# josebeo2016/SCL-Deepfake-audio-detection

Hardware: AMD Instinct MI355X
Metric: train-step utterances/sec (64000-sample clips) (higher is better)
Workload: dtype bf16

## Files before the change

### include/scl_hip.h

```cpp
#ifndef SCL_HIP_H
#define SCL_HIP_H
#include <stdint.h>
#include <stddef.h>

#ifdef __cplusplus
extern "C" {
#endif

#define SCL_OK            0
#define SCL_EINVAL       -1
#define SCL_ELAUNCH      -2
#define SCL_EUNSUPPORTED -3

int         scl_version(void);
const char* scl_last_error(void);

int scl_stream_wait_stream(void* waiter, void* signaler);

#define SCL_KID_GEMM 0
#define SCL_KID_GEMM_F32 2
#define SCL_KID_AUG  1
#define SCL_KID_MAX  8
int scl_build_flags(void);
int scl_prof_enable(int kid, int on);
// ... 45 lines not shown
    const float* bias;
    int64_t c_bs1, c_bs2;
    int64_t c_rbstride;
    int64_t c_split_stride;
    int64_t bias_bs2;
    int32_t c_rpb, ldc;
    int32_t M, N, K;
    int32_t nb1, nb2, splitk;
    int32_t flags;
    float    alpha;
    float    drop_p;
    uint32_t drop_seed;
    int32_t  _pad;
    float*   colsum_part;
} SclGemmDesc;

int scl_gemm_bf16(const SclGemmDesc* desc, void* stream);
int scl_gemm_bf16_group_ok(const SclGemmDesc* descs, int n);
int scl_gemm_bf16_group(const SclGemmDesc* descs, int n, void* stream);
int scl_gemm_bf16_group_tiles(const SclGemmDesc* desc);
int scl_gemm_bf16_group_part(const SclGemmDesc* descs, const int32_t* tile0, const int32_t* ntile, int n, void* stream);

int scl_gemm_uses_wide_tiles(const SclGemmDesc* desc);
int scl_gemm_colsum_rows(const SclGemmDesc* desc);

int scl_posconv_supported(int T, int K, int G, int Cg);
int scl_posconv_wgrad_supported(int T, int K, int G, int Cg);
int scl_posconv_wgrad(const void* dypad, int dy_row0, const void* xpad, float* dw, int B, int T, int K, int G, int Cg, void* stream);
int scl_posconv_mfma(const void* xpad, const void* w, float* C, const float* bias, void* c2, const float* R, int B, int T, int K, int G,
                     int Cg, int fwd, void* stream);

int scl_debug_gemm_stamps(unsigned long long* out, int nblocks);
long long scl_debug_gemm_persistent_launches(void);

int scl_gemm_splitk_finish(const SclGemmDesc* desc, const float* slabs, int nslabs, int64_t stride, void* stream);

int scl_reduce_slabs_f32(const float* slabs, float* out, int64_t n, int nslabs, int64_t stride, void* stream);
#define SCL_SLAB_MAX_JOBS 8
typedef struct SclSlabJob {
    const float* slabs;
    float*       out;
    int64_t      n, stride;
    int32_t      nslabs, _pad;
} SclSlabJob;
int scl_reduce_slabs_multi(const SclSlabJob* jobs, int njobs, void* stream);

int scl_bn_nslabs(int N);
int scl_bn_fwd(const float* x, int N, int C, const float* gamma, const float* beta, float* running_mean, float* running_var,
               long long* num_batches_tracked, int training, float momentum, float eps, int act, float* part, float* mean,
               float* rstd, float* y, void* y2, int y2_bf16, int m_W, int m_HW, int64_t m_bs, int64_t m_rs, int64_t m_cs,
               int64_t m_base, void* stream);
int scl_bn_bwd(const float* dy, const float* y, const float* x, const float* mean, const float* rstd, const float* gamma, int N, int C,
               int act, int training, float* part, float* sums, float* dgamma, float* dbeta, float* dx, int accumulate, void* stream);
int scl_bn_eval_masked(const float* x, int B, int H, int W, int C, const float* gamma, const float* beta, const float* running_mean,
                       const float* running_var, float eps, int act, const int32_t* valid, float* mean, float* rstd, float* y, void* stream);
int scl_bn_eval_cols(const float* x, int B, int H, int W, int C, const float* gamma, const float* beta, const float* running_mean,
                     const float* running_var, float eps, int act, const int32_t* widths, float* mean, float* rstd, float* y, void* stream);
int scl_zero_cols(float* x, int B, int H, int W, int C, const int32_t* widths, void* stream);
int scl_bn_masked_nslabs(int B, int H, int W);
int scl_bn_fwd_masked(const float* x, int B, int H, int W, int C, const float* gamma, const float* beta, float* running_mean,
                      float* running_var, long long* num_batches_tracked, float momentum, float eps, int act, const int32_t* valid,
                      const int32_t* valid_host, float* part, float* mean, float* rstd, float* y, void* stream);
int scl_bn_bwd_masked(const float* dy, const float* y, const float* x, const float* mean, const float* rstd, const float* gamma, int B,
                      int H, int W, int C, int act, const int32_t* valid, const int32_t* valid_host, float* part, float* sums,
                      float* dgamma, float* dbeta, float* dx, int accumulate, void* stream);
int scl_bn_fwd_cols(const float* x, int B, int H, int W, int C, const float* gamma, const float* beta, float* running_mean,
// ... 323 lines not shown
```

### scl-deepfake-audio-detection_amd/csrc/gemm.hip

```cpp
#include "gemm_common.h"

using namespace sclg;

namespace {

constexpr int BM = 128, BN = 128;

struct StageK {
    __amdgpu_buffer_rsrc_t rsrc;
    unsigned rowoff[4];
    unsigned lds_off[4];
    int kcur, kend;

    __device__ __forceinline__ void init(const OpK& o, const char* base, int row0, int rowlimit, int kbegin, int kend_, int tid) {
        rsrc = make_rsrc(base);
        const int c = tid & 7;
#pragma unroll
        for (int i = 0; i < 4; ++i) {
            const int row = (tid >> 3) + 32 * i;
            const int r = row0 + row;
            rowoff[i] = r < rowlimit ? row_off(o, (unsigned)r) : OOB;
            lds_off[i] = (unsigned)(row * 128 + ((c ^ ((row >> 1) & 7)) << 4));
        }
        kcur = kbegin + 8 * c; kend = kend_;
// ... 906 lines not shown
            else SCL_LAUNCH((scl_gemm_big_kernel<true, true>), bgrid, bblock, BIG_LDS, s, k);
#endif
#ifdef SCL_EXPERIMENTS
        } else if (deep) {
            static bool deep_attr_set = false;
            if (!deep_attr_set) {
                hipFuncSetAttribute((const void*)scl_gemm_deep_kernel<false, false, DEEP_S>, hipFuncAttributeMaxDynamicSharedMemorySize, DEEP_LDS);
                hipFuncSetAttribute((const void*)scl_gemm_deep_kernel<false, true, DEEP_S>, hipFuncAttributeMaxDynamicSharedMemorySize, DEEP_LDS);
                hipFuncSetAttribute((const void*)scl_gemm_deep_kernel<true, false, DEEP_S>, hipFuncAttributeMaxDynamicSharedMemorySize, DEEP_LDS);
                hipFuncSetAttribute((const void*)scl_gemm_deep_kernel<true, true, DEEP_S>, hipFuncAttributeMaxDynamicSharedMemorySize, DEEP_LDS);
                deep_attr_set = true;
            }
            if (!at && !bt) SCL_LAUNCH((scl_gemm_deep_kernel<false, false, DEEP_S>), grid, block, DEEP_LDS, s, k);
            else if (!at && bt) SCL_LAUNCH((scl_gemm_deep_kernel<false, true, DEEP_S>), grid, block, DEEP_LDS, s, k);
            else if (at && !bt) SCL_LAUNCH((scl_gemm_deep_kernel<true, false, DEEP_S>), grid, block, DEEP_LDS, s, k);
            else SCL_LAUNCH((scl_gemm_deep_kernel<true, true, DEEP_S>), grid, block, DEEP_LDS, s, k);
#endif
        } else if (dma) {
            if (!at && !bt) SCL_LAUNCH((scl_gemm_dma_kernel<false, false>), grid, block, lds, s, k);
            else if (!at && bt) SCL_LAUNCH((scl_gemm_dma_kernel<false, true>), grid, block, lds, s, k);
            else if (at && !bt) SCL_LAUNCH((scl_gemm_dma_kernel<true, false>), grid, block, lds, s, k);
            else SCL_LAUNCH((scl_gemm_dma_kernel<true, true>), grid, block, lds, s, k);
        } else {
            if (!at && !bt) SCL_LAUNCH((scl_gemm_kernel<false, false>), grid, block, lds, s, k);
            else if (!at && bt) SCL_LAUNCH((scl_gemm_kernel<false, true>), grid, block, lds, s, k);
            else if (at && !bt) SCL_LAUNCH((scl_gemm_kernel<true, false>), grid, block, lds, s, k);
            else SCL_LAUNCH((scl_gemm_kernel<true, true>), grid, block, lds, s, k);
        }
    }
    return scl_check_launch("scl_gemm_bf16");
}

extern "C" long long scl_debug_gemm_persistent_launches(void) { return scl_gemm_w8p_launches(); }
extern "C" int scl_build_flags(void) {
#ifdef SCL_EXPERIMENTS
    return 1;
#else
    return 0;
#endif
}

extern "C" int scl_debug_gemm_stamps(unsigned long long* out, int nblocks) {
    SCL_REQUIRE(out && nblocks > 0 && nblocks <= 4096, "gemm stamps: bad args");
    return scl_gemm_read_stamps(out, nblocks);
}

__global__ __launch_bounds__(256) void scl_gemm_finish_kernel(const GemmK d, const float* __restrict__ slabs, int nslabs, long long stride) {
    const int ncg = (d.N + 3) >> 2;
    const long long idx = (long long)blockIdx.x * 256 + threadIdx.x;
    if (idx >= (long long)d.M * ncg) return;
    const int row = (int)(idx / ncg), col = (int)(idx - (long long)row * ncg) * 4;
    const int flags = d.flags;
    const float* p = slabs + (long long)row * d.N + col;
    float v[4] = {0.f, 0.f, 0.f, 0.f};
    const bool full = col + 4 <= d.N && !(d.N & 3) && !(stride & 3);
    for (int s = 0; s < nslabs; ++s, p += stride) {
        if (full) {
            const float4 t = *reinterpret_cast<const float4*>(p);
            v[0] += t.x; v[1] += t.y; v[2] += t.z; v[3] += t.w;
        } else {
            for (int i = 0; i < 4; ++i) if (col + i < d.N) v[i] += p[i];
        }
    }
    const unsigned q = udiv_magic((unsigned)row, d.c_magic, d.c_shift);
    const long long off = (long long)q * d.c_rbstride + (long long)((unsigned)row - q * d.c_rpb) * d.ldc + col;
    const float* bias = (flags & SCL_GEMM_HAS_BIAS) ? d.bias : nullptr;
// ... 71 lines not shown
```

### scl-deepfake-audio-detection_amd/csrc/gemm_common.h

```cpp
#pragma once
#include "common.h"

namespace sclg {

constexpr int BK = 64;
constexpr int TILE_BYTES = 128 * 64 * 2;
constexpr unsigned OOB = 0xFFFFFFFFu;

struct OpK {
    const void* ptr;
    long long bs1, bs2;
    unsigned rb_bytes, ld_bytes, cout_bytes;
    unsigned rpb, rpb_magic, rpb_shift;
    unsigned cin, cin_magic, cin_mshift, esz_shift;
};
struct GemmK {
    OpK A, B;
    void* C; void* C2; const void* R; const float* bias; float* colsum;
    long long c_bs1, c_bs2, c_rbstride, c_split_stride, bias_bs2;
    unsigned c_rpb, c_magic, c_shift;
    int ldc, M, N, K, nb2, splitk, flags, vec_ok, group_m, tile_m, debug;
    float alpha, drop_p;
    unsigned drop_seed;
};
// ... 226 lines not shown
template <int NMT>
__device__ __forceinline__ void gemm_epilogue_blk(const GemmK& d, f32x4 (&acc)[NMT][4], int mbase, int nbase, int mlimit, int nmt,
                                                  int z1, int z2, int ksplit, int lane) {
    constexpr int KEY = SCL_GEMM_C_F32 | SCL_GEMM_C2_F32 | SCL_GEMM_R_F32 | SCL_GEMM_HAS_BIAS | SCL_GEMM_HAS_C2 | SCL_GEMM_DROPOUT |
                        (0xF << SCL_GEMM_ACT_SHIFT) | (0xF << SCL_GEMM_RMODE_SHIFT) | (0xF << SCL_GEMM_RACT_SHIFT);
    const int f = d.flags & KEY, fb = f & ~SCL_GEMM_HAS_BIAS;
    if (!(d.debug & 16)) {
        if (fb == 0) return gemm_epilogue_blk_k<NMT, 1>(d, acc, mbase, nbase, mlimit, nmt, z1, z2, ksplit, lane);
        if (f == (SCL_GEMM_HAS_BIAS | SCL_GEMM_HAS_C2 | (5 << SCL_GEMM_ACT_SHIFT))) return gemm_epilogue_blk_k<NMT, 2>(d, acc, mbase, nbase, mlimit, nmt, z1, z2, ksplit, lane);
        if (f == ((2 << SCL_GEMM_RMODE_SHIFT) | (4 << SCL_GEMM_RACT_SHIFT))) return gemm_epilogue_blk_k<NMT, 3>(d, acc, mbase, nbase, mlimit, nmt, z1, z2, ksplit, lane);
        if (fb == (SCL_GEMM_C_F32 | SCL_GEMM_R_F32 | (1 << SCL_GEMM_RMODE_SHIFT))) return gemm_epilogue_blk_k<NMT, 4>(d, acc, mbase, nbase, mlimit, nmt, z1, z2, ksplit, lane);
        if (fb == SCL_GEMM_C_F32) return gemm_epilogue_blk_k<NMT, 5>(d, acc, mbase, nbase, mlimit, nmt, z1, z2, ksplit, lane);
    }
    gemm_epilogue_blk_k<NMT, 0>(d, acc, mbase, nbase, mlimit, nmt, z1, z2, ksplit, lane);
}

__device__ __forceinline__ void gemm_epilogue(const GemmK& d, f32x4 (&acc)[4][4], int m0, int n0, int z1, int z2, int ksplit,
                                              int lane, int wr, int wc) {
    gemm_epilogue_blk<4>(d, acc, m0 + wr * 64, n0 + wc * 64, d.M, 4, z1, z2, ksplit, lane);
}





void make_magic(unsigned dv, unsigned* magic, unsigned* shift);
bool fill_operand(const SclOperand& o, const char* name, long long rows, long long contig, OpK* k, int esz);
int scl_gemm_f32_launch(const SclGemmDesc& d, GemmK& k, hipStream_t s);

struct W8Plan { int variant, tiles_m, tile_m; long long tiles, cost; int ncu = 0; };
bool scl_gemm_w8_plan(const GemmK& k, bool at, bool bt, const SclGemmDesc& d, long long zdim, int ncu, W8Plan* plan);
int scl_gemm_read_stamps(unsigned long long* out, int nblocks);
long long scl_gemm_w8p_launches();
int scl_gemm_w8_persist_blocks(const GemmK& k, bool at, bool bt, const W8Plan& plan, long long zdim);
int scl_gemm_w8_launch(GemmK& k, bool at, bool bt, const W8Plan& plan, long long zdim, hipStream_t s);
constexpr int W8_GROUP_MAX = 8;
bool scl_gemm_w8_group_member_ok(const GemmK& k, bool at, bool bt, const SclGemmDesc& d);
int scl_gemm_w8_group_tiles(const GemmK& k);
int scl_gemm_w8_group_launch(GemmK* ks, int n, const int* tile0, const int* ntile, hipStream_t s);

bool scl_gemm_x2_plan(const GemmK& k, bool at, bool bt, const SclGemmDesc& d, long long zdim, int ncu, W8Plan* plan);
int scl_gemm_x2_launch(GemmK& k, bool at, bool bt, const W8Plan& plan, long long zdim, hipStream_t s);

}
```

### scl-deepfake-audio-detection_amd/csrc/gemm_w8.hip

```cpp
#include "gemm_common.h"
#include "gemm_w8_epi.h"

using namespace sclg;

__device__ unsigned long long scl_gemm_stamps[4096 * 8];

namespace {

__device__ __forceinline__ void w8_stamp(const GemmK& d, int slot, int lane, int wave) {
    if ((d.flags & SCL_GEMM_STAMPS) && wave == 0 && lane == 0 && blockIdx.x < 4096 && blockIdx.z == 0) {
        scl_gemm_stamps[blockIdx.x * 8 + 2 * slot] = __builtin_amdgcn_s_memrealtime();
        scl_gemm_stamps[blockIdx.x * 8 + 2 * slot + 1] = __builtin_amdgcn_s_memtime();
    }
}

constexpr int W8_BN = 256;
constexpr int W8_OPB = 2 * TILE_BYTES;
constexpr int W8_NA = 3, W8_NB = 2;
constexpr int W8_LDS = (W8_NA + W8_NB) * W8_OPB;

struct W8K {
    __amdgpu_buffer_rsrc_t rsrc;
    unsigned voff[4];
    __device__ __forceinline__ void init(const OpK& o, const char* base, int row0, int rowlimit, int lane, int wave) {
// ... 321 lines not shown
        __builtin_amdgcn_sched_barrier(0);
        W8S_Q_FIRST(0, 0, RQ0) W8S_Q_FIRST(1, RQ0, RQ1) W8S_Q_FIRST(2, RQ1, RQ2) W8S_Q_FIRST(3, RQ2, NRD)
#undef W8S_Q_FIRST
        lds_wait_upto(0);
        asm volatile("s_waitcnt vmcnt(4)" ::: "memory");
        __builtin_amdgcn_sched_barrier(0);
        __builtin_amdgcn_s_barrier();
        __builtin_amdgcn_sched_barrier(0);
        const char* tBn = bimg + ((kt & 1) ^ 1) * W8_OPB;
#define W8S_B_ISSUE(j) if ((j) < 2) { lb.issue1(tB, wave, soffB, live2b, 2 * (j)); lb.issue1(tB, wave, soffB, live2b, 2 * (j) + 1); }
#define W8S_Q_SECOND(j, R0, R1)                                                                                              \
        RD::template go<R0, R1, false>(fa0, fb0, a_nxt, tBn, ab, nbk, 0, lane);                                              \
        __builtin_amdgcn_sched_barrier(0);                                                                                   \
        _Pragma("unroll") for (int i = 0; i < RBW; ++i)                                                                      \
            acc[i][j] = __builtin_amdgcn_mfma_f32_16x16x32_bf16(fb1[j], fa1[i], acc[i][j], 0, 0, 0);                         \
        __builtin_amdgcn_sched_barrier(0);                                                                                   \
        W8S_B_ISSUE(j)                                                                                                       \
        __builtin_amdgcn_sched_barrier(0);
        W8S_Q_SECOND(0, 0, RQ0) W8S_Q_SECOND(1, RQ0, RQ1) W8S_Q_SECOND(2, RQ1, RQ2) W8S_Q_SECOND(3, RQ2, NRD)
#undef W8S_Q_SECOND
#undef W8S_B_ISSUE
        char* t = a_cur; a_cur = a_nxt; a_nxt = a_fill; a_fill = t;
    }
    asm volatile("s_waitcnt vmcnt(0)" ::: "memory");
    asm volatile("s_waitcnt lgkmcnt(0)" ::: "memory");
    __builtin_amdgcn_s_barrier();
    w8_stamp(d, 2, lane, wave);
    {
        const long long cbase = z1 * d.c_bs1 + z2 * d.c_bs2 + (long long)ksplit * d.c_split_stride;
        const float* bias = (d.flags & SCL_GEMM_HAS_BIAS) ? d.bias + z2 * d.bias_bs2 : nullptr;
        char* wlds = smem + wave * 16384;
        char* wextra = smem + 8 * 16384 + wave * 4096;
        float* cs0 = d.colsum ? d.colsum + ((long long)(m0 / d.tile_m) * 4 + (wave >> 2) * 2) * d.N : nullptr;
        if constexpr (RBW >= 4) {
            f32x4 (&alo)[4][4] = *reinterpret_cast<f32x4 (*)[4][4]>(&acc[0]);
            w8_epilogue_pass<4, ((RBW < 8 && !AT) ? 0x1E : 0)>(d, alo, 4, wlds, wextra, m0 + ab * 16, n0 + wc * 64, mlimit, cbase, bias, lane, cs0);
        } else {
            f32x4 lo[4][4];
#pragma unroll
            for (int i = 0; i < 4; ++i)
#pragma unroll
                for (int j = 0; j < 4; ++j) lo[i][j] = (i < RBW) ? acc[(i < RBW) ? i : 0][j] : f32x4{0.f, 0.f, 0.f, 0.f};
            w8_epilogue_pass<4, ((RBW < 8 && !AT) ? 0x1E : 0)>(d, lo, RBW, wlds, wextra, m0 + ab * 16, n0 + wc * 64, mlimit, cbase, bias, lane, cs0);
        }
        if (RBW > 4) {
            f32x4 hi[4][4];
#pragma unroll
            for (int i = 0; i < 4; ++i)
#pragma unroll
                for (int j = 0; j < 4; ++j) hi[i][j] = (4 + i < RBW) ? acc[(4 + i < RBW) ? 4 + i : 0][j] : f32x4{0.f, 0.f, 0.f, 0.f};
            w8_epilogue_pass<4, ((RBW < 8 && !AT) ? 0x1E : 0)>(d, hi, RBW - 4, wlds, wextra, m0 + (ab + 4) * 16, n0 + wc * 64, mlimit, cbase, bias, lane, cs0 ? cs0 + d.N : nullptr);
        }
    }
    if (d.flags & SCL_GEMM_STAMPS) {
        asm volatile("s_waitcnt vmcnt(0)" ::: "memory");
        w8_stamp(d, 3, lane, wave);
    }
}

template <bool AT, bool BT, int RB0, int RB1, bool SEQ = false>
__device__ __forceinline__ void w8s_tile(const GemmK& d, char* smem, const int bid, const int nblk, const int bz) {
    const int tid = threadIdx.x, lane = tid & 63;
    const int wave = __builtin_amdgcn_readfirstlane(tid >> 6);
    const int wr = wave >> 2, wc = wave & 3;
    w8_stamp(d, 0, lane, wave);
#ifdef SCL_EXPERIMENTS
    if ((d.debug >> 8) && (bid & 1) && bid < 256 && bz == 0) {
        for (int i = 0; i < (d.debug >> 8); ++i) __builtin_amdgcn_s_sleep(127);
    }
#endif
    const int tiles_m = (d.M + d.tile_m - 1) / d.tile_m, tiles_n = (d.N + W8_BN - 1) / W8_BN;
    int tm, tn;
    tile_coords<SEQ>(bid, nblk, tiles_m, tiles_n, tm, tn, d.group_m);
    const int m0 = tm * d.tile_m, n0 = tn * W8_BN;
    const int mlimit = min(d.M, m0 + d.tile_m);
    int z = bz;
    const int ksplit = __builtin_amdgcn_readfirstlane(z % d.splitk); z /= d.splitk;
    const int z1 = __builtin_amdgcn_readfirstlane(z / d.nb2), z2 = z - z1 * d.nb2;
// ... 358 lines not shown
    static bool attr_set = false;
    if (!attr_set) {
        (void)hipFuncSetAttribute((const void*)scl_gemm_w8s_group_kernel<true, true, 8, 8>, hipFuncAttributeMaxDynamicSharedMemorySize, W8_LDS);
        attr_set = true;
    }
    SCL_LAUNCH((scl_gemm_w8s_group_kernel<true, true, 8, 8>), dim3((unsigned)total), dim3(512), W8_LDS, s, g);
    return 0;
}

static long long w8p_launches = 0;
long long scl_gemm_w8p_launches() { return w8p_launches; }

int scl_gemm_read_stamps(unsigned long long* out, int nblocks) {
    return hipMemcpyFromSymbol(out, HIP_SYMBOL(scl_gemm_stamps), sizeof(unsigned long long) * 8 * (size_t)nblocks) == hipSuccess ? 0 : -1;
}

int scl_gemm_w8_persist_blocks(const GemmK& k, bool at, bool bt, const W8Plan& plan, long long zdim) {
    const char* pe = getenv("SCL_W8_PERSIST");
    const int pv = (pe && *pe) ? atoi(pe) : 1;
    const char* me = getenv("SCL_W8_MODE");
    static const bool epi_generic = [] { const char* e = getenv("SCL_W8_EPI_GENERIC"); return e && atoi(e) != 0; }();
    if (pv <= 0 || (me && *me && atoi(me) != 1) || epi_generic) return 0;
    if (plan.variant > 1 || at || zdim != 1 || k.splitk != 1 || k.K / BK < 3 || (k.flags & SCL_GEMM_STAMPS)) return 0;
    const int ek = w8p_epi_kind(k.flags);
    if (!ek || !w8p_built(bt, ek, plan.variant) || ((unsigned)k.flags & SCL_GEMM_C_SPLIT3) || !k.vec_ok || (k.ldc & 7) || (k.c_rbstride & 7)) return 0;
    if (pv >= 8) return pv > 256 ? 256 : (pv & ~7);
    const long long ncu = plan.ncu >= 8 ? plan.ncu : 256;
    const long long rounds = (plan.tiles + ncu - 1) / ncu;
    long long G = (((plan.tiles + rounds - 1) / rounds) + 7) & ~7ll;
    if (G > (ncu & ~7ll)) G = ncu & ~7ll;
    return (G >= 8 && plan.tiles >= 2 * G) ? (int)G : 0;
}

int scl_gemm_w8_launch(GemmK& k, bool at, bool bt, const W8Plan& plan, long long zdim, hipStream_t s) {
    k.tile_m = plan.tile_m;
    k.debug = 0;
    {
        const long long nb1 = zdim / ((long long)k.nb2 * k.splitk);
        const long long rows = k.M - 1, rpb = (long long)k.c_rpb;
        const long long maxoff = (nb1 - 1) * k.c_bs1 + ((long long)k.nb2 - 1) * k.c_bs2 + (rows / rpb) * k.c_rbstride + (rows % rpb) * k.ldc + k.N;
        if (maxoff * ((k.flags & SCL_GEMM_R_F32) ? 4 : 2) >= 0xFFFFFF00ll) k.debug |= 2;
    }
    const dim3 grid((unsigned)plan.tiles, 1, (unsigned)zdim);
    const char* me = getenv("SCL_W8_MODE");
    int mode = (me && *me) ? atoi(me) : 1;
    if (at && bt) {
        if ((long long)k.A.rpb < (long long)k.K) { k.debug |= 4; mode = 0; }
        if ((long long)k.B.rpb < (long long)k.K) { k.debug |= 8; mode = 0; }
    }
    {
        static const bool epi_generic = [] { const char* e = getenv("SCL_W8_EPI_GENERIC"); return e && atoi(e) != 0; }();
        if (epi_generic) k.debug |= 16;
    }
    dim3 g = grid;
#ifdef SCL_EXPERIMENTS
    {
        const char* sg = getenv("SCL_W8_STAGGER");
        const int stg = sg ? atoi(sg) : 0;
        if (stg > 0 && plan.tiles > 256 && zdim == 1) k.debug |= (stg & 0xFF) << 8;
    }
#endif
    if (mode == 1) {
        const int G = scl_gemm_w8_persist_blocks(k, at, bt, plan, zdim);
        if (G > 0) {
            ++w8p_launches;
            w8p_launch(k, bt, w8p_epi_kind(k.flags), plan.variant, dim3((unsigned)G, 1, 1), s);
            return 0;
        }
    }
    if (plan.variant == 2) w8_launch_43(k, bt, g, s);
    else if (plan.variant == 0) w8_launch_rb<7, 6>(k, at, bt, g, s, mode);
    else w8_launch_rb<8, 8>(k, at, bt, g, s, mode);
    return 0;
}

}
```

### scl-deepfake-audio-detection_amd/csrc/gemm_w8_epi.h

```cpp
#pragma once
#include "gemm_common.h"

namespace sclg {

template <int NMT, int EK>
static __device__ __forceinline__ void w8_epilogue_pass_k(const GemmK& d, f32x4 (&acc)[NMT][4], int nmt, char* wlds, char* wextra, int mbase, int nbase,
                                                   int mlimit, long long cbase, const float* bias, int lane, float* csum_row,
                                                   float* cs_carry, const int blk_stride) {
#pragma clang fp contract(off)
    const int flags = d.flags;
    constexpr bool KN = EK != 0;
    const bool c_f32 = KN ? (EK == 4 || EK == 5) : bool(flags & SCL_GEMM_C_F32);
    const bool c2_f32 = KN ? false : bool(flags & SCL_GEMM_C2_F32);
    const bool r_f32 = KN ? (EK == 4) : bool(flags & SCL_GEMM_R_F32);
    const bool has_bias = EK == 2 ? true : (EK == 3 ? false : bool(flags & SCL_GEMM_HAS_BIAS));
    const bool has_c2 = KN ? (EK == 2) : bool(flags & SCL_GEMM_HAS_C2);
    const bool drop = KN ? false : bool(flags & SCL_GEMM_DROPOUT);
    const int act = KN ? (EK == 2 ? 5 : 0) : ((flags >> SCL_GEMM_ACT_SHIFT) & 0xF);
    const int rmode = KN ? (EK == 3 ? 2 : (EK == 4 ? 1 : 0)) : ((flags >> SCL_GEMM_RMODE_SHIFT) & 0xF);
    const int ract = KN ? (EK == 3 ? 4 : 0) : ((flags >> SCL_GEMM_RACT_SHIFT) & 0xF);
    const int g = lane >> 4, lc = lane & 15;
    const int c = lane & 7, rsub = lane >> 3;
    const int col = nbase + 8 * c;
    const bool colv = d.vec_ok && col + 8 <= d.N;
// ... 161 lines not shown
        for (int j = 0; j < 8; ++j) {
            cs[j] += __shfl_xor(cs[j], 8, 64);
            cs[j] += __shfl_xor(cs[j], 16, 64);
            cs[j] += __shfl_xor(cs[j], 32, 64);
        }
        if (lane < 8 && colv) {
            *reinterpret_cast<float4*>(csum_row + col) = make_float4(cs[0], cs[1], cs[2], cs[3]);
            *reinterpret_cast<float4*>(csum_row + col + 4) = make_float4(cs[4], cs[5], cs[6], cs[7]);
        }
    }
}


template <int NMT, int SPEC = 0x1E>
static __device__ __forceinline__ void w8_epilogue_pass(const GemmK& d, f32x4 (&acc)[NMT][4], int nmt, char* wlds, char* wextra, int mbase, int nbase,
                                                 int mlimit, long long cbase, const float* bias, int lane, float* csum_row = nullptr,
                                                 float* cs_carry = nullptr, const int blk_stride = 4096) {
    constexpr int KEY = SCL_GEMM_C_F32 | SCL_GEMM_C2_F32 | SCL_GEMM_R_F32 | SCL_GEMM_HAS_BIAS | SCL_GEMM_HAS_C2 | SCL_GEMM_DROPOUT |
                        (0xF << SCL_GEMM_ACT_SHIFT) | (0xF << SCL_GEMM_RMODE_SHIFT) | (0xF << SCL_GEMM_RACT_SHIFT);
    const int f = d.flags & KEY, fb = f & ~SCL_GEMM_HAS_BIAS;
    if (SPEC != 0 && !(d.debug & 16) && !((unsigned)d.flags & SCL_GEMM_C_SPLIT3) && d.vec_ok && !(d.ldc & 7) && !(d.c_rbstride & 7) && !(cbase & 7)) {
        if ((SPEC & 2) && fb == 0) return w8_epilogue_pass_k<NMT, 1>(d, acc, nmt, wlds, wextra, mbase, nbase, mlimit, cbase, bias, lane, csum_row, cs_carry, blk_stride);
        if ((SPEC & 4) && f == (SCL_GEMM_HAS_BIAS | SCL_GEMM_HAS_C2 | (5 << SCL_GEMM_ACT_SHIFT)))
            return w8_epilogue_pass_k<NMT, 2>(d, acc, nmt, wlds, wextra, mbase, nbase, mlimit, cbase, bias, lane, csum_row, cs_carry, blk_stride);
        if ((SPEC & 8) && f == ((2 << SCL_GEMM_RMODE_SHIFT) | (4 << SCL_GEMM_RACT_SHIFT)))
            return w8_epilogue_pass_k<NMT, 3>(d, acc, nmt, wlds, wextra, mbase, nbase, mlimit, cbase, bias, lane, csum_row, cs_carry, blk_stride);
        if ((SPEC & 16) && fb == (SCL_GEMM_C_F32 | SCL_GEMM_R_F32 | (1 << SCL_GEMM_RMODE_SHIFT)))
            return w8_epilogue_pass_k<NMT, 4>(d, acc, nmt, wlds, wextra, mbase, nbase, mlimit, cbase, bias, lane, csum_row, cs_carry, blk_stride);
        if ((SPEC & 32) && fb == SCL_GEMM_C_F32) return w8_epilogue_pass_k<NMT, 5>(d, acc, nmt, wlds, wextra, mbase, nbase, mlimit, cbase, bias, lane, csum_row, cs_carry, blk_stride);
    }
    w8_epilogue_pass_k<NMT, 0>(d, acc, nmt, wlds, wextra, mbase, nbase, mlimit, cbase, bias, lane, csum_row, cs_carry, blk_stride);
}

static __device__ __forceinline__ void w8_colsum_store(const GemmK& d, float (&cs)[8], float* csum_row, int nbase, int lane) {
    const int col = nbase + 8 * (lane & 7);
#pragma unroll
    for (int j = 0; j < 8; ++j) {
        cs[j] += __shfl_xor(cs[j], 8, 64);
        cs[j] += __shfl_xor(cs[j], 16, 64);
        cs[j] += __shfl_xor(cs[j], 32, 64);
    }
    if (lane < 8 && d.vec_ok && col + 8 <= d.N) {
        *reinterpret_cast<float4*>(csum_row + col) = make_float4(cs[0], cs[1], cs[2], cs[3]);
        *reinterpret_cast<float4*>(csum_row + col + 4) = make_float4(cs[4], cs[5], cs[6], cs[7]);
    }
}

}
```

### scl-deepfake-audio-detection_amd/lib.py

```python
import ctypes
import os

import torch

HERE = os.path.dirname(os.path.abspath(__file__))
LIB_PATH = os.environ.get("SCL_LIB_PATH") or os.path.join(HERE, "libscl_hip.so")
FLAT = 0x7FFFFFFF

_lib = None


class SclError(RuntimeError):
    pass


class SclOperand(ctypes.Structure):
    _fields_ = [("ptr", ctypes.c_void_p), ("bs1", ctypes.c_int64), ("bs2", ctypes.c_int64),
                ("rbstride", ctypes.c_int64), ("cout", ctypes.c_int64), ("rpb", ctypes.c_int32),
                ("ld", ctypes.c_int32), ("cin", ctypes.c_int32), ("_pad", ctypes.c_int32)]


class SclReduceJob(ctypes.Structure):
    _fields_ = [("part", ctypes.c_void_p), ("out", ctypes.c_void_p), ("out2", ctypes.c_void_p), ("pstride", ctypes.c_int64),
                ("nparts", ctypes.c_int32), ("C", ctypes.c_int32), ("split", ctypes.c_int32), ("_pad", ctypes.c_int32)]
# ... 60 lines not shown
ACT_NONE, ACT_GELU, ACT_RELU, ACT_LEAKY = 0, 1, 2, 3
ACT_GELU_DC2 = 5
RACT_STORED = 4
KID_GEMM = 0
KID_AUG = 1
KID_GEMM_F32 = 2

_vp, _i32, _i64, _f32, _f64, _u32 = (ctypes.c_void_p, ctypes.c_int32, ctypes.c_int64, ctypes.c_float,
                                     ctypes.c_double, ctypes.c_uint32)


def _protos():
    P = ctypes.POINTER
    return {
        "scl_version": ([], _i32),
        "scl_last_error": ([], ctypes.c_char_p),
        "scl_build_flags": ([], _i32),
        "scl_prof_enable": ([_i32, _i32], _i32),
        "scl_prof_reserve": ([_i32, _i32], _i32),
        "scl_prof_read": ([_i32, P(_i64), P(_f64), P(_f64)], _i32),
        "scl_prof_read_launches": ([_i32, _i32, P(ctypes.c_float), P(_i32), P(_i64)], _i32),
        "scl_gemm_bf16": ([P(SclGemmDesc), _vp], _i32),
        "scl_gemm_bf16_group_ok": ([P(SclGemmDesc), _i32], _i32),
        "scl_gemm_bf16_group": ([P(SclGemmDesc), _i32, _vp], _i32),
        "scl_gemm_bf16_group_tiles": ([P(SclGemmDesc)], _i32),
        "scl_gemm_bf16_group_part": ([P(SclGemmDesc), P(_i32), P(_i32), _i32, _vp], _i32),
        "scl_reduce_slabs_f32": ([_vp, _vp, _i64, _i32, _i64, _vp], _i32),
        "scl_posconv_supported": ([_i32, _i32, _i32, _i32], _i32),
        "scl_posconv_wgrad_supported": ([_i32, _i32, _i32, _i32], _i32),
        "scl_posconv_wgrad": ([_vp, _i32, _vp, _vp, _i32, _i32, _i32, _i32, _i32, _vp], _i32),
        "scl_posconv_mfma": ([_vp, _vp, _vp, _vp, _vp, _vp, _i32, _i32, _i32, _i32, _i32, _i32, _vp], _i32),
        "scl_debug_gemm_stamps": ([_vp, _i32], _i32),
        "scl_debug_gemm_persistent_launches": ([], ctypes.c_longlong),
        "scl_gemm_uses_wide_tiles": ([P(SclGemmDesc)], _i32),
        "scl_gemm_colsum_rows": ([P(SclGemmDesc)], _i32),
        "scl_bn_nslabs": ([_i32], _i32),
        "scl_bn_fwd": ([_vp, _i32, _i32, _vp, _vp, _vp, _vp, _vp, _i32, _f32, _f32, _i32, _vp, _vp, _vp, _vp, _vp, _i32, _i32, _i32, _i64, _i64,
                        _i64, _i64, _vp], _i32),
        "scl_bn_bwd": ([_vp, _vp, _vp, _vp, _vp, _vp, _i32, _i32, _i32, _i32, _vp, _vp, _vp, _vp, _vp, _i32, _vp], _i32),
        "scl_bn_eval_masked": ([_vp, _i32, _i32, _i32, _i32, _vp, _vp, _vp, _vp, _f32, _i32, _vp, _vp, _vp, _vp, _vp], _i32),
        "scl_bn_eval_cols": ([_vp, _i32, _i32, _i32, _i32, _vp, _vp, _vp, _vp, _f32, _i32, _vp, _vp, _vp, _vp, _vp], _i32),
        "scl_zero_cols": ([_vp, _i32, _i32, _i32, _i32, _vp, _vp], _i32),
        "scl_pad_nhwc_f32": ([_vp, _i64, _i32, _vp, _i32, _i32, _i32, _i64, _i64, _i64, _i64, _vp], _i32),
        "scl_conv_pack_weights": ([_vp, _vp, _vp, _i32, _i32, _i32, _i32, _i32, _i32, _vp], _i32),
        "scl_conv_wgrad_finish": ([_vp, _vp, _i32, _i32, _i32, _i32, _i32, _i32, _i32, _vp], _i32),
        "scl_maxpool3_fwd": ([_vp, _i64, _i64, _i64, _i32, _i32, _i32, _vp, _vp, _vp], _i32),
        "scl_maxpool3_bwd": ([_vp, _vp, _i32, _i32, _i32, _vp, _i64, _i64, _i64, _vp], _i32),
        "scl_avgpool_fwd": ([_vp, _i32, _i32, _i32, _vp, _vp], _i32),
        "scl_avgpool_bwd": ([_vp, _i32, _i32, _i32, _vp, _vp], _i32),
        "scl_avgpool_fwd_masked": ([_vp, _vp, _i32, _i32, _i32, _i32, _vp, _vp], _i32),
        "scl_bn_masked_nslabs": ([_i32, _i32, _i32], _i32),
        "scl_bn_fwd_masked": ([_vp, _i32, _i32, _i32, _i32, _vp, _vp, _vp, _vp, _vp, _f32, _f32, _i32, _vp, _vp, _vp, _vp, _vp, _vp, _vp], _i32),
        "scl_bn_bwd_masked": ([_vp, _vp, _vp, _vp, _vp, _vp, _i32, _i32, _i32, _i32, _i32, _vp, _vp, _vp, _vp, _vp, _vp, _vp, _i32, _vp], _i32),
        "scl_bn_fwd_cols": ([_vp, _i32, _i32, _i32, _i32, _vp, _vp, _vp, _vp, _vp, _f32, _f32, _i32, _vp, _vp, _vp, _vp, _vp, _vp, _vp], _i32),
        "scl_bn_bwd_cols": ([_vp, _vp, _vp, _vp, _vp, _vp, _i32, _i32, _i32, _i32, _i32, _vp, _vp, _vp, _vp, _vp, _vp, _vp, _i32, _vp], _i32),
        "scl_avgpool_bwd_masked": ([_vp, _vp, _vp, _i32, _i32, _i32, _i32, _vp, _vp], _i32),
        "scl_layernorm_fwd": ([_vp, _i32, _vp, _vp, _vp, _vp, _vp, _vp, _i32, _i32, _i64, _i64, _f32, _i32, _vp], _i32),
        "scl_layernorm_bwd_nparts": ([_i32], _i32),
        "scl_layernorm_bwd": ([_vp, _i32, _vp, _i32, _vp, _vp, _vp, _vp, _vp, _vp, _vp, _vp, _i32, _i32, _i64, _i64,
                               _i64, _i32, _i32, _i32, _i64, _i64, _u32, _f32, _u32, _f32, _vp], _i32),
        "scl_colreduce_f32": ([_vp, _vp, _i32, _i32, _i64, _i32, _vp], _i32),
        "scl_colsum_nparts": ([_i32], _i32),
        "scl_colsum_reduce_nparts": ([_i32, _i32], _i32),
        "scl_colsum": ([_vp, _i32, _vp, _i32, _i32, _i64, _vp], _i32),
        "scl_colreduce_multi": ([P(SclReduceJob), _i32, _vp], _i32),
        "scl_reduce_slabs_multi": ([P(SclSlabJob), _i32, _vp], _i32),
# ... 223 lines not shown
```

Baseline: 1697.

## Prefetch residual operand into LDS ahead of GEMM epilogue stores

Adds a specialized w8 GEMM epilogue for the residual-add (f32) and residual-multiply (bf16) fusion kinds. It issues async buffer-to-LDS loads of the R tile a couple of row groups ahead, so the residual reads overlap the accumulator staging and output stores instead of stalling each row. The path is enabled by default through an env-gated host check that sets a debug flag, with strict alignment and flag conditions. It adds hand-written waitcnt sequencing and extra LDS traffic, which could hurt if the vmcnt accounting or the LDS slot reuse is off.

```diff
diff --git a/include/scl_hip.h b/include/scl_hip.h
--- a/include/scl_hip.h
+++ b/include/scl_hip.h
@@ -101,6 +101,7 @@
 
 int scl_debug_gemm_stamps(unsigned long long* out, int nblocks);
 long long scl_debug_gemm_persistent_launches(void);
+long long scl_debug_gemm_r_ahead_launches(void);
 
 int scl_gemm_splitk_finish(const SclGemmDesc* desc, const float* slabs, int nslabs, int64_t stride, void* stream);
 
diff --git a/scl-deepfake-audio-detection_amd/csrc/gemm.hip b/scl-deepfake-audio-detection_amd/csrc/gemm.hip
--- a/scl-deepfake-audio-detection_amd/csrc/gemm.hip
+++ b/scl-deepfake-audio-detection_amd/csrc/gemm.hip
@@ -962,6 +962,7 @@
 }
 
 extern "C" long long scl_debug_gemm_persistent_launches(void) { return scl_gemm_w8p_launches(); }
+extern "C" long long scl_debug_gemm_r_ahead_launches(void) { return scl_gemm_w8_r_ahead_launches(); }
 extern "C" int scl_build_flags(void) {
 #ifdef SCL_EXPERIMENTS
     return 1;
diff --git a/scl-deepfake-audio-detection_amd/csrc/gemm_common.h b/scl-deepfake-audio-detection_amd/csrc/gemm_common.h
--- a/scl-deepfake-audio-detection_amd/csrc/gemm_common.h
+++ b/scl-deepfake-audio-detection_amd/csrc/gemm_common.h
@@ -282,6 +282,7 @@
 bool scl_gemm_w8_plan(const GemmK& k, bool at, bool bt, const SclGemmDesc& d, long long zdim, int ncu, W8Plan* plan);
 int scl_gemm_read_stamps(unsigned long long* out, int nblocks);
 long long scl_gemm_w8p_launches();
+long long scl_gemm_w8_r_ahead_launches();
 int scl_gemm_w8_persist_blocks(const GemmK& k, bool at, bool bt, const W8Plan& plan, long long zdim);
 int scl_gemm_w8_launch(GemmK& k, bool at, bool bt, const W8Plan& plan, long long zdim, hipStream_t s);
 constexpr int W8_GROUP_MAX = 8;
diff --git a/scl-deepfake-audio-detection_amd/csrc/gemm_w8.hip b/scl-deepfake-audio-detection_amd/csrc/gemm_w8.hip
--- a/scl-deepfake-audio-detection_amd/csrc/gemm_w8.hip
+++ b/scl-deepfake-audio-detection_amd/csrc/gemm_w8.hip
@@ -377,7 +377,21 @@
         char* wlds = smem + wave * 16384;
         char* wextra = smem + 8 * 16384 + wave * 4096;
         float* cs0 = d.colsum ? d.colsum + ((long long)(m0 / d.tile_m) * 4 + (wave >> 2) * 2) * d.N : nullptr;
-        if constexpr (RBW >= 4) {
+        const int ahead = (RBW < 8 && !AT) ? w8_epi_ahead_kind(d, cbase) : 0;
+        if (ahead) {
+            f32x4 lo[4][4], hi[4][4];
+#pragma unroll
+            for (int i = 0; i < 4; ++i)
+#pragma unroll
+                for (int j = 0; j < 4; ++j) {
+                    lo[i][j] = (i < RBW) ? acc[(i < RBW) ? i : 0][j] : f32x4{0.f, 0.f, 0.f, 0.f};
+                    hi[i][j] = (4 + i < RBW) ? acc[(4 + i < RBW) ? 4 + i : 0][j] : f32x4{0.f, 0.f, 0.f, 0.f};
+                }
+            constexpr int NLO = RBW < 4 ? RBW : 4, NHI = RBW > 4 ? RBW - 4 : 0;
+            const int mb0 = m0 + ab * 16, mb1 = m0 + (ab + 4) * 16, nb = n0 + wc * 64;
+            if (ahead == 3) w8_epilogue_ahead<3, (RBW > 4)>(d, lo, NLO, hi, NHI, wlds, wextra, mb0, mb1, nb, mlimit, cbase, bias, lane, cs0, 4096);
+            else w8_epilogue_ahead<4, (RBW > 4)>(d, lo, NLO, hi, NHI, wlds, wextra, mb0, mb1, nb, mlimit, cbase, bias, lane, cs0, 4096);
+        } else if constexpr (RBW >= 4) {
             f32x4 (&alo)[4][4] = *reinterpret_cast<f32x4 (*)[4][4]>(&acc[0]);
             w8_epilogue_pass<4, ((RBW < 8 && !AT) ? 0x1E : 0)>(d, alo, 4, wlds, wextra, m0 + ab * 16, n0 + wc * 64, mlimit, cbase, bias, lane, cs0);
         } else {
@@ -388,7 +402,7 @@
                 for (int j = 0; j < 4; ++j) lo[i][j] = (i < RBW) ? acc[(i < RBW) ? i : 0][j] : f32x4{0.f, 0.f, 0.f, 0.f};
             w8_epilogue_pass<4, ((RBW < 8 && !AT) ? 0x1E : 0)>(d, lo, RBW, wlds, wextra, m0 + ab * 16, n0 + wc * 64, mlimit, cbase, bias, lane, cs0);
         }
-        if (RBW > 4) {
+        if (RBW > 4 && !ahead) {
             f32x4 hi[4][4];
 #pragma unroll
             for (int i = 0; i < 4; ++i)
@@ -813,6 +827,21 @@
     return (G >= 8 && plan.tiles >= 2 * G) ? (int)G : 0;
 }
 
+constexpr int W8_R_AHEAD_KINDS = 1 << 3;
+static long long w8_r_ahead_launches = 0;
+long long scl_gemm_w8_r_ahead_launches() { return w8_r_ahead_launches; }
+static bool scl_gemm_w8_r_ahead(const GemmK& k, bool at, const W8Plan& plan, int mode) {
+    const char* e = getenv("SCL_W8_R_AHEAD");
+    const int v = (e && *e) ? atoi(e) : 1;
+    const int kinds = v <= 0 ? 0 : (v == 1 ? W8_R_AHEAD_KINDS : v);
+    const int f = k.flags & W8_EPI_KEY;
+    const int ek = f == ((2 << SCL_GEMM_RMODE_SHIFT) | (4 << SCL_GEMM_RACT_SHIFT)) ? 3
+                 : ((f & ~SCL_GEMM_HAS_BIAS) == (SCL_GEMM_C_F32 | SCL_GEMM_R_F32 | (1 << SCL_GEMM_RMODE_SHIFT)) ? 4 : 0);
+    if (!ek || !((kinds >> ek) & 1) || at || mode != 1 || plan.variant == 1 || (k.debug & (2 | 16)) || ((unsigned)k.flags & SCL_GEMM_C_SPLIT3)) return false;
+    if (!k.vec_ok || (k.N & 7) || (k.ldc & 7) || (k.c_rbstride & 7) || (k.c_bs1 & 7) || (k.c_bs2 & 7) || (k.c_split_stride & 7)) return false;
+    return ((((uintptr_t)k.R) | ((uintptr_t)k.C)) & 15) == 0;
+}
+
 int scl_gemm_w8_launch(GemmK& k, bool at, bool bt, const W8Plan& plan, long long zdim, hipStream_t s) {
     k.tile_m = plan.tile_m;
     k.debug = 0;
@@ -849,6 +878,10 @@
             return 0;
         }
     }
+    if (scl_gemm_w8_r_ahead(k, at, plan, mode)) {
+        k.debug |= 32;
+        ++w8_r_ahead_launches;
+    }
     if (plan.variant == 2) w8_launch_43(k, bt, g, s);
     else if (plan.variant == 0) w8_launch_rb<7, 6>(k, at, bt, g, s, mode);
     else w8_launch_rb<8, 8>(k, at, bt, g, s, mode);
diff --git a/scl-deepfake-audio-detection_amd/csrc/gemm_w8_epi.h b/scl-deepfake-audio-detection_amd/csrc/gemm_w8_epi.h
--- a/scl-deepfake-audio-detection_amd/csrc/gemm_w8_epi.h
+++ b/scl-deepfake-audio-detection_amd/csrc/gemm_w8_epi.h
@@ -217,6 +217,146 @@
     w8_epilogue_pass_k<NMT, 0>(d, acc, nmt, wlds, wextra, mbase, nbase, mlimit, cbase, bias, lane, csum_row, cs_carry, blk_stride);
 }
 
+static __device__ __forceinline__ int w8_epi_ahead_kind(const GemmK& d, long long cbase) {
+    constexpr int KEY = SCL_GEMM_C_F32 | SCL_GEMM_C2_F32 | SCL_GEMM_R_F32 | SCL_GEMM_HAS_BIAS | SCL_GEMM_HAS_C2 | SCL_GEMM_DROPOUT |
+                        (0xF << SCL_GEMM_ACT_SHIFT) | (0xF << SCL_GEMM_RMODE_SHIFT) | (0xF << SCL_GEMM_RACT_SHIFT);
+    if ((d.debug & (32 | 16 | 2)) != 32 || ((unsigned)d.flags & SCL_GEMM_C_SPLIT3) || !d.vec_ok || (d.ldc & 7) || (d.c_rbstride & 7) || (cbase & 7) || (d.N & 7) ||
+        (((unsigned long long)d.R | (unsigned long long)d.C) & 15))
+        return 0;
+    const int f = d.flags & KEY;
+    if (f == ((2 << SCL_GEMM_RMODE_SHIFT) | (4 << SCL_GEMM_RACT_SHIFT))) return 3;
+    if ((f & ~SCL_GEMM_HAS_BIAS) == (SCL_GEMM_C_F32 | SCL_GEMM_R_F32 | (1 << SCL_GEMM_RMODE_SHIFT))) return 4;
+    return 0;
+}
+
+static __device__ __forceinline__ void lds_write16_raw(const char* p, f32x4 v) {
+    const unsigned a = (unsigned)(uintptr_t)(lds_void*)(p);
+    asm volatile("ds_write_b128 %0, %1" ::"v"(a), "v"(v) : "memory");
+}
+static __device__ __forceinline__ f32x4 lds_read16_raw(const char* p) {
+    const unsigned a = (unsigned)(uintptr_t)(lds_void*)(p);
+    f32x4 v;
+    asm volatile("ds_read_b128 %0, %1" : "=&v"(v) : "v"(a) : "memory");
+    return v;
+}
+
+template <int EK, bool TWO>
+static __device__ __forceinline__ void w8_epilogue_ahead(const GemmK& d, f32x4 (&lo)[4][4], int nlo, f32x4 (&hi)[4][4], int nhi, char* wlds, char* wextra,
+                                                  int mbase0, int mbase1, int nbase, int mlimit, long long cbase, const float* bias, int lane,
+                                                  float* csum_row, const int blk_stride) {
+#pragma clang fp contract(off)
+    static_assert(EK == 3 || EK == 4, "w8_epilogue_ahead: the kinds with an R operand");
+    constexpr bool r_f32 = EK == 4;
+    constexpr int ESH = r_f32 ? 2 : 1;
+    constexpr int RG = r_f32 ? 2048 : 1024;
+    constexpr int NL = r_f32 ? 2 : 1, NS = NL;
+    const bool has_bias = EK == 4 && (d.flags & SCL_GEMM_HAS_BIAS);
+    const int g = lane >> 4, lc = lane & 15;
+    const int c = lane & 7, rsub = lane >> 3;
+    const int col = nbase + 8 * c;
+    const bool colv = col + 8 <= d.N;
+    const __amdgpu_buffer_rsrc_t r_rsrc = make_rsrc(reinterpret_cast<const char*>(d.R));
+    const __amdgpu_buffer_rsrc_t c_rsrc = make_rsrc(reinterpret_cast<const char*>(d.C));
+    auto offb = [&](int row) {
+        const unsigned q = udiv_magic((unsigned)row, d.c_magic, d.c_shift);
+        const long long o = cbase + (long long)q * d.c_rbstride + (long long)((unsigned)row - q * d.c_rpb) * d.ldc + col;
+        return (row < mlimit && colv) ? (unsigned)(o << ESH) : OOB;
+    };
+    auto r_request = [&](char* dst, int row) {
+        const unsigned o = offb(row);
+        __builtin_amdgcn_raw_ptr_buffer_load_lds(r_rsrc, (lds_void*)dst, 16, o, 0, 0, 0);
+        if (r_f32) __builtin_amdgcn_raw_ptr_buffer_load_lds(r_rsrc, (lds_void*)(dst + 1024), 16, o == OOB ? OOB : o + 16, 0, 0, 0);
+    };
+    float bb[8] = {0.f, 0.f, 0.f, 0.f, 0.f, 0.f, 0.f, 0.f};
+    if (has_bias && colv) {
+        const float4 b0 = *reinterpret_cast<const float4*>(bias + col), b1 = *reinterpret_cast<const float4*>(bias + col + 4);
+        bb[0] = b0.x; bb[1] = b0.y; bb[2] = b0.z; bb[3] = b0.w; bb[4] = b1.x; bb[5] = b1.y; bb[6] = b1.z; bb[7] = b1.w;
+    }
+    r_request(wextra, mbase0 + rsub);
+    r_request(wextra + RG, mbase0 + 8 + rsub);
+    auto pass = [&](f32x4 (&acc)[4][4], const int nmt, const int mbase, float* cs_row, const bool first, const int mnext) {
+#pragma unroll
+        for (int mt = 0; mt < 4; ++mt) {
+            if (mt < nmt) {
+#pragma unroll
+                for (int nt = 0; nt < 4; ++nt) lds_write16_raw(wlds + mt * blk_stride + lc * 256 + (((nt * 4 + g) ^ lc) << 4), acc[mt][nt]);
+            }
+        }
+        float cs[8] = {0.f, 0.f, 0.f, 0.f, 0.f, 0.f, 0.f, 0.f};
+        const int ng = 2 * nmt;
+#pragma nounroll
+        for (int i = 0; i < ng; ++i) {
+            if (first && i == 0) asm volatile("s_waitcnt vmcnt(%0)" ::"n"(NL) : "memory");
+            else if (mnext < 0 && i == ng - 1) asm volatile("s_waitcnt vmcnt(%0)" ::"n"(NS) : "memory");
+            else asm volatile("s_waitcnt vmcnt(%0)" ::"n"(NS + NL) : "memory");
+            char* const slot = wlds + (i >> 1) * blk_stride + (i & 1) * 2048;
+            const char* rst = (i < 2 ? wextra + i * RG : wlds + ((i - 2) >> 1) * blk_stride + (i & 1) * 2048) + lane * 16;
+            const int r = 8 * i + rsub;
+            const char* wrow = slot + rsub * 256;
+            f32x4 alo = lds_read16_raw(wrow + (((2 * c) ^ (r & 15)) << 4));
+            f32x4 ahi = lds_read16_raw(wrow + (((2 * c + 1) ^ (r & 15)) << 4));
+            f32x4 t0 = lds_read16_raw(rst), t1 = t0;
+            if (r_f32) {
+                t1 = lds_read16_raw(rst + 1024);
+                asm volatile("s_waitcnt lgkmcnt(0)" : "+v"(alo), "+v"(ahi), "+v"(t0), "+v"(t1)::"memory");
+            } else {
+                asm volatile("s_waitcnt lgkmcnt(0)" : "+v"(alo), "+v"(ahi), "+v"(t0)::"memory");
+            }
+            float rr[8];
+            if (r_f32) {
+                rr[0] = t0[0]; rr[1] = t0[1]; rr[2] = t0[2]; rr[3] = t0[3]; rr[4] = t1[0]; rr[5] = t1[1]; rr[6] = t1[2]; rr[7] = t1[3];
+            } else {
+                const unsigned tx = __float_as_uint(t0[0]), ty = __float_as_uint(t0[1]), tz = __float_as_uint(t0[2]), tw = __float_as_uint(t0[3]);
+                rr[0] = __uint_as_float(tx << 16); rr[1] = __uint_as_float(tx & 0xFFFF0000u);
+                rr[2] = __uint_as_float(ty << 16); rr[3] = __uint_as_float(ty & 0xFFFF0000u);
+                rr[4] = __uint_as_float(tz << 16); rr[5] = __uint_as_float(tz & 0xFFFF0000u);
+                rr[6] = __uint_as_float(tw << 16); rr[7] = __uint_as_float(tw & 0xFFFF0000u);
+            }
+            const int row = mbase + r;
+            const unsigned ob = offb(row);
+            float v[8] = {d.alpha * alo[0], d.alpha * alo[1], d.alpha * alo[2], d.alpha * alo[3], d.alpha * ahi[0], d.alpha * ahi[1], d.alpha * ahi[2], d.alpha * ahi[3]};
+            if (has_bias) {
+#pragma unroll
+                for (int j = 0; j < 8; ++j) v[j] += bb[j];
+            }
+            if (r_f32) {
+#pragma unroll
+                for (int j = 0; j < 8; ++j) v[j] += rr[j];
+            } else {
+#pragma unroll
+                for (int j = 0; j < 8; ++j) v[j] *= rr[j];
+            }
+            if (cs_row) {
+#pragma unroll
+                for (int j = 0; j < 8; ++j) cs[j] = ob != OOB ? cs[j] + v[j] : cs[j];
+            }
+            if (r_f32) {
+                __builtin_amdgcn_raw_buffer_store_b128(u32x4{__float_as_uint(v[0]), __float_as_uint(v[1]), __float_as_uint(v[2]), __float_as_uint(v[3])}, c_rsrc, ob, 0, 0);
+                __builtin_amdgcn_raw_buffer_store_b128(u32x4{__float_as_uint(v[4]), __float_as_uint(v[5]), __float_as_uint(v[6]), __float_as_uint(v[7])}, c_rsrc, ob == OOB ? OOB : ob + 16, 0, 0);
+            } else {
+                __builtin_amdgcn_raw_buffer_store_b128(u32x4{pack_bf2(v[0], v[1]), pack_bf2(v[2], v[3]), pack_bf2(v[4], v[5]), pack_bf2(v[6], v[7])}, c_rsrc, ob, 0, 0);
+            }
+            const int j2 = i + 2;
+            if (j2 < ng) r_request(slot, mbase + 8 * j2 + rsub);
+            else if (mnext >= 0) r_request(wextra + (j2 - ng) * RG, mnext + 8 * (j2 - ng) + rsub);
+        }
+        if (cs_row) {
+#pragma unroll
+            for (int j = 0; j < 8; ++j) {
+                cs[j] += __shfl_xor(cs[j], 8, 64);
+                cs[j] += __shfl_xor(cs[j], 16, 64);
+                cs[j] += __shfl_xor(cs[j], 32, 64);
+            }
+            if (lane < 8 && colv) {
+                *reinterpret_cast<float4*>(cs_row + col) = make_float4(cs[0], cs[1], cs[2], cs[3]);
+                *reinterpret_cast<float4*>(cs_row + col + 4) = make_float4(cs[4], cs[5], cs[6], cs[7]);
+            }
+        }
+    };
+    pass(lo, nlo, mbase0, csum_row, true, TWO ? mbase1 : -1);
+    if (TWO) pass(hi, nhi, mbase1, csum_row ? csum_row + d.N : nullptr, false, -1);
+}
+
 static __device__ __forceinline__ void w8_colsum_store(const GemmK& d, float (&cs)[8], float* csum_row, int nbase, int lane) {
     const int col = nbase + 8 * (lane & 7);
 #pragma unroll
diff --git a/scl-deepfake-audio-detection_amd/lib.py b/scl-deepfake-audio-detection_amd/lib.py
--- a/scl-deepfake-audio-detection_amd/lib.py
+++ b/scl-deepfake-audio-detection_amd/lib.py
@@ -116,6 +116,7 @@
         "scl_posconv_mfma": ([_vp, _vp, _vp, _vp, _vp, _vp, _i32, _i32, _i32, _i32, _i32, _i32, _vp], _i32),
         "scl_debug_gemm_stamps": ([_vp, _i32], _i32),
         "scl_debug_gemm_persistent_launches": ([], ctypes.c_longlong),
+        "scl_debug_gemm_r_ahead_launches": ([], ctypes.c_longlong),
         "scl_gemm_uses_wide_tiles": ([P(SclGemmDesc)], _i32),
         "scl_gemm_colsum_rows": ([P(SclGemmDesc)], _i32),
         "scl_bn_nslabs": ([_i32], _i32),
```

Measured after the change: 1699 (median of 5 runs). No clear change (+0.1%).
